# BradenDKelly/MetropolisMonteCarlo

Hardware: AMD Instinct MI355X
Metric: MC trial moves/sec (whole node), SPC/E NVT full Ewald fp64 (higher is better)
Workload: dtype f64

## Files before the change

### metropolismontecarlo_amd/csrc/mmc_batch.inc

```

#include <atomic>
#include <chrono>
#include <cmath>
#include <thread>

#define MMC_MAX_GROUPS 64
#define MMC_SERVER_AUTO_MAX 256
#define MMC_GEN_MAX 16
#define MMC_GEN_RING (MMC_GEN_MAX + 2)

struct mmc_batch {
    DeviceSystem sys;
    double lj_rcut = 0, qq_rcut = 0;
    int n_parts = 1;
    int kernel = 3;
    int server_wgs = -1;
    int wave_wgs = 0;
    int n_cus = 256;
    bool fast_ok = false;
    bool rigid_only = true;
    int image_by_molecule = -1;
    int zero_copy_moves = 0;
    MoveRec *h_moves[2] = { nullptr, nullptr };
    MoveRec *hd_moves[2] = { nullptr, nullptr };
    MoveRec *d_moves[2] = { nullptr, nullptr };
    PartOut *h_parts = nullptr, *d_parts = nullptr;
    int32_t *h_accept = nullptr, *d_accept = nullptr;
    int32_t *dev_accept = nullptr;
    int buf = 0;
    bool has_prev = false;
    std::vector<uint8_t> s_cur;
    std::vector<double> h_com, h_at;
    bool mirror_valid = false;
    int device_moves = 0;
    MoveRec *d_ring = nullptr;
    double *d_quat = nullptr;
    unsigned stamp = 0;
    int64_t steps_done = 0;
    int eval_parts = 0;
    int quat_mode = 0;
    double db[9] = { 0 };
    int persistent = -1;
    unsigned long long *h_ctrl = nullptr, *hd_ctrl = nullptr;
    unsigned long long *bar_ctrl = nullptr;
    int32_t *h_timeout = nullptr, *hd_timeout = nullptr;
    hipStream_t run_streams[MMC_MAX_GROUPS] = {};
    hipEvent_t run_events[MMC_MAX_GROUPS][4] = {};
    void *pool = nullptr;
    void (*pool_destroy)(void *) = nullptr;
    int steps_per_launch = 0;
    int accept_on_device = -1;
    DecideConsts *d_decide = nullptr;
    DecideConsts decide_host{};
    int server_stall_ms = 0;
    int64_t server_seq_offset = 0;
    bool needs_reload = false;
    std::vector<uint8_t> reloaded;
    int inject_torn = 0;
    bool vol_outstanding = false;
    bool vol_saved_fast_ok = false;
    int vol_saved_kernel = 0;
    std::vector<int32_t> pb_moved;
    int64_t trace_steps = 0;
    std::vector<double> trace_delta;
    std::vector<uint8_t> trace_flags;
    uint8_t *h_flags = nullptr, *hd_flags = nullptr, *d_flags = nullptr;
    uint8_t *bar_flags = nullptr;
    double2 *h_steps = nullptr, *hd_steps = nullptr, *d_steps = nullptr;
    void *widom_buf = nullptr;
    size_t widom_bytes = 0;
    void *widom_host = nullptr;
    size_t widom_host_bytes = 0;

    const MoveRec *dev_moves(int which) const
    {
        return zero_copy_moves ? hd_moves[which] : d_moves[which];
    }
};

static int32_t batch_pinned(void **h, void **d, size_t bytes)
{
    MMC_HIP(hipHostMalloc(h, bytes, hipHostMallocMapped | hipHostMallocCoherent));
    MMC_HIP(hipHostGetDevicePointer(d, *h, 0));
    memset(*h, 0, bytes);
    return MMC_OK;
}
// ... 167 lines not shown
        MMC_REQUIRE(value >= 0 && value <= (1 << 20), MMC_ERR_ARG, "wave_wgs outside 0..2^20");
        b->wave_wgs = (int)value;
    } else if (!strcmp(key, "server_wgs")) {
        MMC_REQUIRE(value >= -1 && value <= LAT_MAX_PARTS / LAT_WAVES && value != 1, MMC_ERR_ARG,
                    "server_wgs must be -1 (choose), 0 (one workgroup per replica) or 2..%d",
                    LAT_MAX_PARTS / LAT_WAVES);
        b->server_wgs = (int)value;
    } else if (!strcmp(key, "persistent")) {
        MMC_REQUIRE(value >= -1 && value <= 1, MMC_ERR_ARG, "persistent must be -1, 0 or 1");
        MMC_REQUIRE(!b->sys.pb.on || value != 1, MMC_ERR_UNSUPPORTED,
                    "per-replica boxes: the move server has one box");
        b->persistent = (int)value;
    } else if (!strcmp(key, "server_seq_offset")) {
        MMC_REQUIRE(value >= 0, MMC_ERR_ARG, "server_seq_offset must be >= 0");
        b->server_seq_offset = value;
    } else if (!strcmp(key, "server_stall_ms")) {
        MMC_REQUIRE(value >= 0 && value <= 10000, MMC_ERR_ARG, "server_stall_ms outside 0..10000");
        b->server_stall_ms = (int)value;
    } else if (!strcmp(key, "inject_torn")) {
        b->inject_torn = (int)value;
    } else if (!strcmp(key, "trace_steps")) {
        MMC_REQUIRE(value >= 0 && value * b->sys.R <= (1LL << 26), MMC_ERR_ARG, "trace_steps out of range");
        b->trace_steps = value;
    } else if (!strcmp(key, "zero_copy_moves")) {
        b->zero_copy_moves = value ? 1 : 0;
    } else if (!strcmp(key, "device_moves")) {
        MMC_REQUIRE(!b->sys.pb.on || value, MMC_ERR_UNSUPPORTED,
                    "per-replica boxes: the trial moves are drawn on the device");
        b->device_moves = value ? 1 : 0;
    } else if (!strcmp(key, "steps_per_launch")) {
        MMC_REQUIRE(value == 0 || value == 1 || value == 2 || value == 4 || value == 8 || value == 16, MMC_ERR_ARG,
                    "steps_per_launch must be 0 (by size), 1, 2, 4, 8 or 16");
        b->steps_per_launch = (int)value;
    } else if (!strcmp(key, "accept_on_device")) {
        MMC_REQUIRE(value >= -1 && value <= 1, MMC_ERR_ARG, "accept_on_device must be -1 (by size), 0 (host) or 1 (kernel)");
        b->accept_on_device = (int)value;
    } else if (!strcmp(key, "image_by_molecule")) {
        MMC_REQUIRE(value == -1 || value == 0, MMC_ERR_ARG, "image_by_molecule must be -1 (where valid) or 0 (never)");
        b->image_by_molecule = (int)value;
    } else {
        mmc_set_error("unknown option '%s'", key);
        return MMC_ERR_ARG;
    }
    return MMC_OK;
}

extern "C" int32_t mmc_batch_set_parts(mmc_batch *b, int32_t n_parts)
{
    return mmc_batch_set_option(b, "parts", n_parts);
}

extern "C" int32_t mmc_batch_set_replica(mmc_batch *b, int64_t r, const double *com,
                                         const double *coords)
{
    BATCH_CHECK(b);
    MMC_REQUIRE(!b->has_prev, MMC_ERR_STATE, "proposals outstanding: call mmc_batch_settle first");
    BATCH_NO_VOLUME_TRIAL(b);
    MMC_REQUIRE(com && coords, MMC_ERR_ARG, "NULL array argument");
    MMC_TRY(b->sys.set_replica(r, com, coords));
    if (b->needs_reload) {
        b->reloaded[r] = 1;
        bool all = true;
        for (uint8_t v : b->reloaded) all = all && v;
        if (all) {
            b->needs_reload = false;
            b->s_cur.assign(b->sys.R, 0);
// ... 46 lines not shown
    const int64_t n_mol = b->sys.n_mol;
    b->h_com.resize((size_t)b->sys.R * n_mol * 3);
    b->h_at.resize((size_t)b->sys.R * n_mol * 9);
    for (int64_t r = 0; r < b->sys.R; r++)
        MMC_TRY(b->sys.get_replica(r, &b->h_com[(size_t)r * n_mol * 3],
                                   &b->h_at[(size_t)r * n_mol * 9]));
    b->mirror_valid = true;
    return MMC_OK;
}

static inline void batch_mirror_commit(mmc_batch *b, int64_t r, const MoveRec &m)
{
    const int64_t n_mol = b->sys.n_mol;
    memcpy(&b->h_com[((size_t)r * n_mol + (m.mol - 1)) * 3], m.com_new, sizeof(double) * 3);
    memcpy(&b->h_at[((size_t)r * n_mol + (m.mol - 1)) * 9], m.atoms_new, sizeof(double) * 9);
}

static inline void batch_fill_old(mmc_batch *b, int64_t r, MoveRec &m)
{
    const int64_t n_mol = b->sys.n_mol;
    memcpy(m.com_old, &b->h_com[((size_t)r * n_mol + (m.mol - 1)) * 3], sizeof(double) * 3);
    memcpy(m.atoms_old, &b->h_at[((size_t)r * n_mol + (m.mol - 1)) * 9], sizeof(double) * 9);
}

struct DevGen {
    uint64_t seed;
    uint64_t replica0;
    int64_t rng_off;
    int64_t step;
    int n_gen;
    bool upload_steps;
};

static int32_t batch_ensure_ring(mmc_batch *b)
{
    if (!b->d_ring)
        MMC_TRY(b->sys.dmalloc((void **)&b->d_ring, sizeof(MoveRec) * MMC_GEN_RING * b->sys.R));
    return MMC_OK;
}

static inline const MoveRec *batch_ring_slot(const mmc_batch *b, int64_t step)
{
    return b->d_ring + (step % MMC_GEN_RING) * b->sys.R;
}

static int batch_kernel_for(const mmc_batch *b, int64_t nr, int P)
{
    if (b->sys.pb.on)
        return 1;
    return b->kernel != 3 ? b->kernel : (nr * P >= (int64_t)16 * b->n_cus ? 2 : 1);
}

struct DevDecide {
    const DecideConsts *dc;
    int64_t step;
    PartOut *parts;
    bool fetch_flags;
    int n_sub;
};

static int32_t batch_launch(mmc_batch *b, hipStream_t stream, int64_t r0, int64_t nr, int P,
                            int buf, bool has_prev, const PairParams &pp,
                            hipEvent_t before_kernel = nullptr, const DevGen *dg = nullptr,
                            unsigned stamp = 0, const DevDecide *dd = nullptr)
{
    DeviceSystem &s = b->sys;
    const MoveRec *cur, *prev;
    const uint8_t *flagv = nullptr;
    if (dg) {
        flagv = b->hd_flags;
        const double2 *stp = b->hd_steps;
        if (!b->zero_copy_moves) {
            if (dd ? dd->fetch_flags : !b->bar_flags)
                k_fetch_bytes<<<(unsigned)((nr + 1023) / 1024), 256, 0, stream>>>(
                    b->d_flags + r0, b->hd_flags + r0, (int)nr);
            if (dg->upload_steps)
                MMC_HIP(hipMemcpyAsync(b->d_steps + r0, b->h_steps + r0, sizeof(double2) * nr,
                                       hipMemcpyHostToDevice, stream));
            flagv = b->bar_flags && !dd ? b->bar_flags : b->d_flags;
            stp = b->d_steps;
        }
        if (dg->n_gen > 0) {
            GenArgs ga;
            ga.steps = stp; ga.seed = dg->seed; ga.replica0 = dg->replica0;
            ga.rng_off = dg->rng_off; ga.step0 = dg->step; ga.n_gen = dg->n_gen;
            ga.ring = MMC_GEN_RING; ga.ring_stride = s.R; ga.flag0 = flagv;
            ga.quat_mode = b->quat_mode;
            memcpy(ga.db, b->db, sizeof(ga.db));
            const int64_t n = nr * dg->n_gen;
            if (s.pb.on)
                k_propose<<<(unsigned)((n + 63) / 64), 64, 0, stream>>>(s.bv, s.rec, b->d_ring, ga, (int)r0,
                                                                        (int)nr, has_prev ? 1 : 0, s.pb_view());
            else
                k_propose<<<(unsigned)((n + 63) / 64), 64, 0, stream>>>(s.bv, s.rec, b->d_ring, ga,
                                                                        (int)r0, (int)nr, has_prev ? 1 : 0);
        }
        cur = batch_ring_slot(b, dg->step);
        prev = has_prev ? batch_ring_slot(b, dg->step + MMC_GEN_RING - 1) : nullptr;
    } else {
        b->rigid_only = false;
        s.r_mol_max = INFINITY;
        if (!b->zero_copy_moves)
            MMC_HIP(hipMemcpyAsync(b->d_moves[buf] + r0, b->h_moves[buf] + r0,
                                   sizeof(MoveRec) * nr, hipMemcpyHostToDevice, stream));
        cur = b->dev_moves(buf);
        prev = has_prev ? b->dev_moves(buf ^ 1) : nullptr;
    }
    if (before_kernel)
        MMC_HIP(hipEventRecord(before_kernel, stream));
    dim3 grid((unsigned)P, (unsigned)nr);
    MMC_REQUIRE(!dd || (dg && P == 1 && !b->zero_copy_moves && batch_kernel_for(b, nr, P) == 2), MMC_ERR_ASSERT,
                "the kernel's own accept decision needs device-side proposals, one part per move and the wave kernel");
    const int kernel = batch_kernel_for(b, nr, P);
    if (kernel == 4) {
        MMC_REQUIRE(lat_applies(4 * P, (int)s.n_mol, (int)s.nkvecs), MMC_ERR_UNSUPPORTED,
                    "kernel 4 needs 4..%d parts (a multiple of 4) with at most %d molecules per pair "
                    "part", LAT_MAX_PARTS, LAT_MAXMOL);
        k_move_eval_lat<<<grid, LAT_WAVES * 64, 0, stream>>>(s.bv, s.rec, s.qq_tab, s.kpack, s.fc,
                                                             cur, prev, b->d_parts, 4 * P, pp, (int)r0,
                                                             flagv, stamp);
    } else if (kernel == 2) {
        const int64_t n_units = nr * P;
        int64_t wgs = (n_units + WV_MWAVES - 1) / WV_MWAVES;
        const int64_t cap = b->wave_wgs > 0 ? b->wave_wgs : (int64_t)(4 * WV_OCC / WV_MWAVES) * b->n_cus;
        if (wgs > cap) wgs = cap;
        const bool img = dg && b->rigid_only && b->image_by_molecule != 0 &&
                         s.image_by_molecule(std::max(pp.lj_gate_sq, pp.qq_gate_sq)) &&
                         s.pairs_inside_slack(pp.qq_gate_sq, pp.qq_slack_sq) &&
                         s.pairs_inside_slack(pp.lj_gate_sq, pp.lj_slack_sq);
#define MMC_WAVE_LAUNCH(SUBST, IMG) MMC_WAVE_LAUNCH3(SUBST, IMG, false)
#define MMC_WAVE_LAUNCH3(SUBST, IMG, MULTI)                                                      \
    k_move_eval_wave<SUBST, IMG, MULTI><<<(unsigned)wgs, WV_MWAVES * 64, 0, stream>>>(            \
        s.bv, s.rec, s.qq_tab, s.kpack, s.fc, cur, prev, dd ? dd->parts : b->d_parts, P, pp,     \
        (int)r0, (int)n_units, flagv, stamp, dd ? dd->dc : nullptr, dd ? (long long)dd->step : 0LL,      \
        dd ? dd->n_sub : 1, (int)(dg ? dg->step % MMC_GEN_RING : 0))
        if (P == 1 && dd && dd->n_sub > 1) {
            if (img) MMC_WAVE_LAUNCH3(false, true, true); else MMC_WAVE_LAUNCH3(false, false, true);
        } else if (P == 1) {
            if (img) MMC_WAVE_LAUNCH(false, true); else MMC_WAVE_LAUNCH(false, false);
        } else {
            if (img) MMC_WAVE_LAUNCH(true, true); else MMC_WAVE_LAUNCH(true, false);
        }
#undef MMC_WAVE_LAUNCH
#undef MMC_WAVE_LAUNCH3
    } else if (kernel == 1 && s.pb.on)
        k_move_eval_fast<<<grid, MMC_BLOCK, 0, stream>>>(s.bv, s.rec, nullptr, s.kpack, s.fc, cur, prev,
                                                         b->d_parts, P, pp, (int)r0, flagv, stamp,
                                                         s.pb_view());
    else if (kernel == 1)
        k_move_eval_fast<<<grid, MMC_BLOCK, 0, stream>>>(s.bv, s.rec, s.qq_tab, s.kpack, s.fc, cur,
                                                         prev, b->d_parts, P, pp, (int)r0, flagv,
                                                         stamp);
    else
        k_move_eval<<<grid, MMC_BLOCK, 0, stream>>>(s.bv, cur, prev, b->d_parts, P, pp, (int)r0,
                                                    s.rec, flagv, stamp);
    MMC_HIP(hipGetLastError());
    return MMC_OK;
}

static int batch_server_parts(int64_t n_mol, int64_t R)
{
    int64_t pairs = (n_mol + 63) / 64;
    const int64_t cap = R == 1 ? 4 : SRV_WAVES - 1;
    if (pairs > cap) pairs = cap;
    if (pairs < 1) pairs = 1;
    return (int)pairs + 1;
}

// ... 421 lines not shown
```

### metropolismontecarlo_amd/csrc/mmc_engine.inc

```
#include <atomic>
#include <chrono>
#include <cmath>
#include <condition_variable>
#include <mutex>
#include <thread>

#ifndef MMC_HOST_CHUNK
#define MMC_HOST_CHUNK 128
#endif

namespace {

struct Rng {
    uint64_t s[4];
    static uint64_t splitmix(uint64_t &x)
    {
        uint64_t z = (x += 0x9e3779b97f4a7c15ULL);
        z = (z ^ (z >> 30)) * 0xbf58476d1ce4e5b9ULL;
        z = (z ^ (z >> 27)) * 0x94d049bb133111ebULL;
        return z ^ (z >> 31);
    }
    void seed(uint64_t v)
    {
        for (int k = 0; k < 4; k++)
// ... 96 lines not shown
    std::chrono::steady_clock::time_point t_post;
};

inline void adjust_step(int64_t &naccepp, int64_t &attempp, int64_t naccept, int64_t attempt,
                        double set_value, double L, double &d_max)
{
    if (attempp == 0) {
        naccepp = naccept;
        attempp = attempt;
        return;
    }
    if (attempt == attempp)
        return;
    const double ratio = (double)(naccept - naccepp) / (double)(attempt - attempp);
    const double dr_old = d_max;
    d_max = d_max * ratio / set_value;
    const double dr_ratio = d_max / dr_old;
    if (dr_ratio > 1.5) d_max = dr_old * 1.5;
    if (dr_ratio < 0.5) d_max = dr_old * 0.5;
    if (d_max > L / 2) d_max = L / 2;
    naccepp = naccept;
    attempp = attempt;
}

struct Driver {
    mmc_batch *b;
    const mmc_run_params *p;
    double *energies;
    mmc_chain *chains = nullptr;
    int adjust = 0;
    bool devgen = false;
    bool devacc = false;
    int K = 1;
    bool server = false;
    int server_waves = 0;
    int server_lat_wgs = 0;
    std::vector<Group> groups;
    std::vector<Rng> rng;
    std::vector<uint8_t> acc_prev, kind;
    PairParams pp;
    int P = 1, T = 1;
    SpinBarrier bar;
    std::atomic<int32_t> status{ MMC_OK };
    std::atomic<int> drained_polls{ 0 };
    char err[256] = "";
    std::vector<mmc_run_stats> tstats;
    std::vector<double> trace_t;
    std::chrono::steady_clock::time_point trace_t0;
    std::vector<double> entry_t;
    std::vector<double> mark_t;
    double now_us() const { return std::chrono::duration<double, std::micro>(std::chrono::steady_clock::now() - trace_t0).count(); }
    int64_t rng_off = 0;
    std::atomic<int> inject_left{ 0 };

    ChainKey chain_key(int64_t r) const
    {
        return ChainKey{ p->seed, (uint32_t)(p->replica0 + (uint64_t)r) };
    }

    int collect(int64_t r, unsigned want, PartOut *parts, int &q_done, mmc_run_stats &st, int slot = 0)
    {
        for (; q_done < P; q_done++) {
            const PartOut *src = &b->h_parts[(size_t)slot * b->sys.R + r * P + q_done];
            if (part_stamp_of(*(const volatile int32_t *)&src->ovl[1]) != want)
                return 0;
            std::atomic_thread_fence(std::memory_order_acquire);
// ... 84 lines not shown
                        c.rot_set_value, b->sys.box, c.dphi_max);
            if (devgen)
                b->h_steps[r] = make_double2(c.dr_max, c.dphi_max);
        }
    }

    void metropolis(const Group &g, int64_t lo, int64_t hi, int64_t step_done, mmc_run_stats &st,
                    bool gated = false, int slot = -1)
    {
        const unsigned want = (slot >= 0 ? g.stamp_of[slot] : g.stamp) & MMC_STAMP_MASK;
        const int sl = slot >= 0 ? slot : 0;
        if (gated && hi > lo) {
            const PartOut *gate = &b->h_parts[(size_t)sl * b->sys.R + (hi - 1) * P + (P - 1)];
            for (unsigned spins = 1; part_stamp_of(*(const volatile int32_t *)&gate->ovl[1]) != want; spins++) {
                if (((spins & 0xffff) == 0 && !still_running(g)) || status.load(std::memory_order_relaxed) != MMC_OK)
                    return;
                for (int k = 0; k < 16; k++)
                    mmc_cpu_relax();
            }
        }
        for (int64_t r = lo; r < hi; r++) {
            PartOut parts[MMC_MAX_PARTS];
            int q_done = 0;
            for (unsigned spins = 1;; spins++) {
                const int c = collect(r, want, parts, q_done, st, sl);
                if (c > 0)
                    break;
                if (c < 0 || ((spins & 0xfffff) == 0 && !still_running(g)))
                    return;
                mmc_cpu_relax();
            }
            const int64_t n_sub = slot >= 0 ? std::min<int64_t>(K, p->n_steps - step_done) : 1;
            if (n_sub > 1) {
                unsigned long long bits;
                memcpy(&bits, &parts[0].lj_pot[1], 8);
                const unsigned acc_mask = (unsigned)bits & 0xffffu, ovl_mask = (unsigned)(bits >> 16) & 0xffffu,
                               kind_mask = (unsigned)(bits >> 32) & 0xffffu;
                energies[r] += parts[0].lj_pot[0];
                for (int64_t k = 0; k < n_sub; k++) {
                    const int kd = (kind_mask >> k) & 1;
                    const bool acc = (acc_mask >> k) & 1;
                    if (kd == 0) { st.trans_attempt++; st.trans_accept += acc; }
                    else { st.rot_attempt++; st.rot_accept += acc; }
                    st.overlaps += (ovl_mask >> k) & 1;
                    if (acc && step_done + k + 1 < p->n_steps)
                        b->s_cur[r] ^= 1;
                    if (k + 1 == n_sub) {
                        acc_prev[r] = acc ? 1 : 0;
                        kind[r] = (uint8_t)kd;
                    }
                }
                st.moves += n_sub;
            } else if (slot >= 0) {
                kind[r] = (uint8_t)mmc_move_kind(chain_key(r), (uint64_t)(rng_off + step_done));
                decide(r, parts, step_done, st, part_accept_of(parts[0].ovl[1]));
                if (acc_prev[r] && step_done + 1 < p->n_steps)
                    b->s_cur[r] ^= 1;
            } else
                decide(r, parts, step_done, st);
        }
    }

    template <class F> void share(const Group &g, int t, F &&fn) const
    {
        const int64_t tail = g.nr >= 16 * (int64_t)MMC_HOST_CHUNK * T && !no_tail_share ? g.nr / tail_div : 0;
        const int64_t bulk = g.nr - tail;
        if (bulk * t / T < bulk * (t + 1) / T)
            fn(g.r0 + bulk * t / T, g.r0 + bulk * (t + 1) / T, false);
        const int64_t n_chunks = (tail + MMC_HOST_CHUNK - 1) / MMC_HOST_CHUNK;
        for (int64_t c = t; c < n_chunks; c += T) {
// ... 94 lines not shown
            timed = false;
        }
        return MMC_OK;
    }

    int32_t launch(Group &g, int64_t step, mmc_run_stats &st, hipStream_t on = nullptr)
    {
        g.launched_on = on ? on : g.stream;
        if (server) {
            const bool new_steps = step == 0 || (adjust && step % b->sys.n_mol == 0);
            g.n_launch++;
            g.timed = false;
            g.stamp = ++b->stamp;
            g.t_post = std::chrono::steady_clock::now();
            std::atomic_thread_fence(std::memory_order_release);
            if (b->server_stall_ms > 0 && step == 2)
                std::this_thread::sleep_for(std::chrono::milliseconds(b->server_stall_ms));
            for (int64_t r = g.r0; r < g.r0 + g.nr; r++)
                batch_server_post(b, r, step + 1, g.stamp,
                                  (unsigned)b->h_flags[r] | (new_steps ? SRV_STEPS : 0u));
            st.launches++;
            return MMC_OK;
        }
        DevGen dg{};
        if (devgen) {
            const int64_t n_mol = b->sys.n_mol, i0 = step % n_mol;
            dg.seed = p->seed;
            dg.replica0 = p->replica0;
            dg.rng_off = rng_off;
            dg.step = step;
            dg.upload_steps = step == 0 || (adjust && i0 == 0);
            if (step >= g.gen_end) {
                int64_t k = n_mol - 1 < 1 ? 1 : n_mol - 1;
                if (k > MMC_GEN_MAX) k = MMC_GEN_MAX;
                if (k > p->n_steps - step) k = p->n_steps - step;
                if (adjust && k > n_mol - i0) k = n_mol - i0;
                dg.n_gen = (int)k;
                g.gen_end = step + k;
            }
        }
        g.n_launch++;
        g.timed = p->time_kernels > 0
                  && (g.n_launch - 1) % (unsigned)p->time_kernels == (unsigned)p->time_kernels / 2;
        g.stamp = ++b->stamp;
        if (devacc) {
            const int64_t n_sub = std::min<int64_t>(K, p->n_steps - step);
            const int slot = (int)((step / K) & 1);
            g.stamp_of[slot] = g.stamp;
            g.timed_of[slot] = g.timed;
            DevDecide dd{ b->d_decide, rng_off + step, b->d_parts + (size_t)slot * b->sys.R, step == 0, (int)n_sub };
            MMC_TRY(batch_launch(b, g.launched_on, g.r0, g.nr, P, g.buf, step > 0, pp,
                                 g.timed ? g.evs[slot][0] : nullptr, &dg, g.stamp, &dd));
            if (g.timed)
                MMC_HIP(hipEventRecord(g.evs[slot][1], g.launched_on));
            g.timed = false;
            st.launches++;
            return MMC_OK;
        }
        MMC_TRY(batch_launch(b, g.launched_on, g.r0, g.nr, P, g.buf, g.has_prev, pp,
                             g.timed ? g.ev0 : nullptr, devgen ? &dg : nullptr, g.stamp));
        if (g.timed)
            MMC_HIP(hipEventRecord(g.ev1, g.launched_on));
        st.launches++;
        return MMC_OK;
    }

    void settle_slice(const Group &g, int64_t lo, int64_t hi)
    {
        const MoveRec *prev = b->h_moves[g.buf];
        for (int64_t r = lo; r < hi; r++) {
            b->h_accept[r] = acc_prev[r];
            if (acc_prev[r]) {
                b->s_cur[r] ^= 1;
                if (!devgen)
                    batch_mirror_commit(b, r, prev[r]);
            }
        }
    }
    int32_t settle_enqueue(Group &g)
    {
        return batch_settle_range(b, g.stream, g.r0, g.nr,
                                  devgen ? batch_ring_slot(b, p->n_steps - 1) : b->dev_moves(g.buf), false);
    }
// ... 454 lines not shown
        }
        if (p->time_kernels) {
            for (int k = 0; k < 4; k++)
                if (!b->run_events[g][k])
                    MMC_HIP(hipEventCreate(&b->run_events[g][k]));
            d.groups[g].ev0 = b->run_events[g][0];
            d.groups[g].ev1 = b->run_events[g][1];
            for (int k = 0; k < 4; k++)
                d.groups[g].evs[k / 2][k % 2] = b->run_events[g][k];
        }
    }
    d.devacc = d.devgen && !d.server && d.P == 1 && !b->zero_copy_moves && !(chains && adjust);
    int64_t nr_max = 0;
    for (const Group &g : d.groups) {
        d.devacc = d.devacc && batch_kernel_for(b, g.nr, d.P) == 2;
        nr_max = std::max(nr_max, g.nr);
    }
    {
        int want = b->accept_on_device;
        if (getenv("MMC_DEVICE_ACCEPT")) want = 1;
        if (getenv("MMC_HOST_ACCEPT")) want = 0;
        const bool multi_ok = !chains && b->trace_steps == 0 && s.n_mol > MMC_GEN_MAX && b->steps_per_launch != 1;
        if (want < 0)
            want = (multi_ok || nr_max > (int64_t)4096 * d.T) ? 1 : 0;
        d.devacc = d.devacc && want == 1;
    }
    d.K = 1;
    if (d.devacc && !chains && b->trace_steps == 0 && s.n_mol > MMC_GEN_MAX) {
        d.K = b->steps_per_launch > 0 ? b->steps_per_launch : 8;
        if (const char *e = getenv("MMC_STEPS_PER_LAUNCH"))
            d.K = atoi(e);
        if (d.K != 1 && d.K != 2 && d.K != 4 && d.K != 8 && d.K != 16)
            d.K = 1;
    }
    if (d.devacc) {
        MMC_TRY(batch_ensure_ring(b));
        DecideConsts dc{};
        dc.temperature = p->temperature; dc.factor = s.bv.factor;
        dc.seed = p->seed; dc.replica0 = (uint32_t)p->replica0;
        dc.flags = b->d_flags;
        dc.ring = b->d_ring; dc.ring_slots = MMC_GEN_RING; dc.ring_stride = s.R;
        if (!b->d_decide)
            MMC_TRY(s.dmalloc((void **)&b->d_decide, sizeof(DecideConsts)));
        if (memcmp(&dc, &b->decide_host, sizeof(dc)) != 0) {
            MMC_HIP(hipMemcpy(b->d_decide, &dc, sizeof(dc), hipMemcpyHostToDevice));
            b->decide_host = dc;
        }
        if (const char *e = getenv("MMC_RUN_AHEAD"))
            d.run_ahead = atoi(e) ? 1 : 0;
        if (const char *e = getenv("MMC_LAUNCH_AT"))
            d.launch_at = std::min(1.0, std::max(0.0, atof(e) / 100.0));
    }
    if (d.server)
        for (Group &g : d.groups)
            g.stream = d.groups[0].stream;
    if (d.server)
        MMC_TRY(batch_server_start(b, d.groups[0].stream, d.server_waves, d.pp, p->seed, p->replica0,
                                   b->steps_done, d.server_lat_wgs));
    d.rng.resize(d.devgen ? 0 : R);
    for (int64_t r = 0; r < (d.devgen ? 0 : R); r++) {
        uint64_t h = p->seed;
        h = Rng::splitmix(h) ^ (p->replica0 + (uint64_t)r);
        h = Rng::splitmix(h) ^ (uint64_t)b->steps_done;
        d.rng[r].seed(h);
    }
    d.acc_prev.assign(R, 0);
    d.kind.assign(R, 0);
    b->trace_delta.assign((size_t)(b->trace_steps * R), 0.0);
    b->trace_flags.assign((size_t)(b->trace_steps * R), 0);
    d.tstats.assign(d.T, mmc_run_stats{});
    if (d.server) {
        d.server_stamp0 = b->stamp;
        b->stamp += (unsigned)p->n_steps;
    }

    const auto t0 = std::chrono::steady_clock::now();
// ... 74 lines not shown
    }
    stats->server_steps = d.server ? p->n_steps : 0;
    stats->device_decisions = d.devacc ? stats->moves : 0;
    if (d.server)
        stats->launches = p->n_steps * (int64_t)d.groups.size();
    stats->wall_ms = std::chrono::duration<double, std::milli>(t1 - t0).count();
    for (int64_t r = 0; r < R; r++)
        stats->energy_sum += chains ? chains[r].energy : energies[r];
    for (size_t g = 0; g < d.groups.size(); g++)
        if (d.groups[g].stream)
            (void)hipStreamSynchronize(d.groups[g].stream);
    if (run_trace) {
        const auto t2 = std::chrono::steady_clock::now();
        auto us = [](std::chrono::steady_clock::duration x) { return std::chrono::duration<double, std::micro>(x).count(); };
        fprintf(stderr, "run trace: threads %.0f us, final settle %.0f us (enqueued after %.0f), last sync %.0f us; launches at",
                us(t_join - t_enter), us(t1 - t_join), us(t_enq - t_join), us(t2 - t1));
        for (double x : d.trace_t)
            fprintf(stderr, " %.0f", x);
        fprintf(stderr, "\nrun trace: threads entered at");
        for (double x : d.entry_t)
            fprintf(stderr, " %.0f", x);
        fprintf(stderr, "\nrun trace: thread 0 per (step, group) [after barrier, after its share, (same), after barrier]:");
        for (size_t k = 0; k < d.mark_t.size(); k++)
            fprintf(stderr, "%s%.0f", k % 4 == 0 ? " | " : " ", d.mark_t[k]);
        fprintf(stderr, "\n");
    }
    b->buf = 0;
    b->has_prev = false;
    b->inject_torn = 0;
    if (status == MMC_OK)
        b->steps_done += p->n_steps;
    else {
        b->needs_reload = true;
        b->reloaded.assign(R, 0);
    }
    return status;
}

extern "C" int32_t mmc_batch_run(mmc_batch *b, const mmc_run_params *p, double *energies,
                                 mmc_run_stats *stats)
{
    MMC_REQUIRE(energies, MMC_ERR_ARG, "NULL argument");
    return run_impl(b, p, energies, nullptr, 0, stats);
}

extern "C" int32_t mmc_batch_run_chains(mmc_batch *b, const mmc_run_params *p, mmc_chain *chains,
                                        int32_t adjust, mmc_run_stats *stats)
{
    MMC_REQUIRE(chains, MMC_ERR_ARG, "NULL argument");
    if (b)
        BATCH_ONE_BOX(b, "mmc_batch_run_chains");
    if (b)
        for (int64_t r = 0; r < b->sys.R; r++)
            MMC_REQUIRE(chains[r].dr_max >= 0 && chains[r].dphi_max >= 0
                            && (!adjust || (chains[r].trans_set_value > 0 && chains[r].rot_set_value > 0)),
                        MMC_ERR_ARG, "chain %lld: bad step sizes / set values", (long long)r);
    return run_impl(b, p, nullptr, chains, adjust, stats);
}

extern "C" int32_t mmc_batch_run_npt(mmc_batch *b, const mmc_run_params *p, const mmc_npt_params *q,
                                     double *energy, mmc_run_stats *stats, mmc_npt_stats *ns)
{
    BATCH_CHECK(b);
    BATCH_ONE_BOX(b, "mmc_batch_run_npt (per-replica boxes: mmc_batch_run_npt_replicas)");
    MMC_REQUIRE(p && q && energy && stats && ns, MMC_ERR_ARG, "NULL argument");
    MMC_REQUIRE(b->sys.R == 1, MMC_ERR_UNSUPPORTED,
// ... 89 lines not shown
```

### metropolismontecarlo_amd/csrc/mmc_kernels.hpp

```cpp
#pragma once
#include "mmc_device.hpp"

struct BatchView {
    double *comx, *comy, *comz;
    double *ax, *ay, *az;
    int64_t mol_stride, atom_stride;
    const int32_t *first0, *cnt, *atype;
    const double *charge, *eps, *sig;
    int32_t n_mol, n_atoms, n_types;
    double box;
    double *S;
    int64_t nk_stride;
    const int32_t *kxyz;
    const double *cfac;
    const int16_t *kmap;
    int32_t nkvecs, nk;
    double kappa, factor;
    uint16_t *comq;
    int64_t cq_stride;
    double *quat;
};

__host__ __device__ inline uint16_t com_quant(double x, double inv_box)
{
// ... 360 lines not shown
    h += dpp_row_shr<2>(h);
    h += dpp_row_shr<4>(h);
    return part_checksum_fold((uint32_t)__builtin_amdgcn_readlane(h, 7));
}

__device__ inline double pack_ovl(int o0, int o1, unsigned stamp, uint32_t csum, int accept = 0)
{
    const unsigned lo = (csum << 1) | (unsigned)(o0 & 1),
                   hi = ((unsigned)(accept & 1) << 31) | ((stamp & MMC_STAMP_MASK) << 1) | (unsigned)(o1 & 1);
    return __longlong_as_double((long long)(((unsigned long long)hi << 32) | lo));
}
__host__ __device__ inline uint32_t part_stamp_of(int32_t ovl1) { return ((uint32_t)ovl1 >> 1) & MMC_STAMP_MASK; }
__host__ __device__ inline int part_accept_of(int32_t ovl1) { return (int)((uint32_t)ovl1 >> 31); }

__host__ __device__ inline double mmc_move_delta(const double *w7, bool ov_old, bool ov_new, double factor)
{
    const double e0 = (0.0 + w7[0]) * 4, e1 = (0.0 + w7[1]) * 4;
    double q0 = ov_old ? 0.0 : 0.0 + w7[4], q1 = ov_new ? 0.0 : 0.0 + w7[5];
    q0 *= factor; q1 *= factor;
    const double d_recip = (ov_old || ov_new) ? 0.0 : (0.0 + w7[6]) * factor;
    return ((e1 - e0) + (q1 - q0)) + d_recip;
}

struct MoveRec;
struct DecideConsts {
    double temperature, factor;
    uint64_t seed;
    uint32_t replica0;
    int32_t ring_slots;
    const MoveRec *ring;
    int64_t ring_stride;
    uint8_t *flags;
};
#define MMC_STEPS_PER_LAUNCH_MAX 16

__global__ __launch_bounds__(MMC_BLOCK) void k_move_eval(BatchView bv, const MoveRec *cur,
                                                         const MoveRec *prev, PartOut *out,
                                                         int n_parts, PairParams pp, int r_base,
                                                         double *rec, const uint8_t *flagv,
                                                         unsigned stamp)
{
    __shared__ __align__(16) double pobuf[8];
    __shared__ Chosen ch;
    __shared__ Pending pd;
    __shared__ int32_t list[MMC_LIST_CAP];
    __shared__ int32_t wcnt[MMC_WAVES];
    __shared__ double red[6 * MMC_WAVES];
    __shared__ cplx tab[2][3][3][MMC_NKTAB];

    const int r = r_base + blockIdx.y, part = blockIdx.x, tid = threadIdx.x;
    const SysView s = sys_view(bv, r);
    const MoveRec *mv = cur + r;
    const int flags = flagv ? (int)flagv[r] : mv->flags;
    const bool commit = prev && (flags & 1);
    const int scur = (flags >> 1) & 1;
    const int i0 = mv->mol - 1;
    const int pend = commit ? prev[r].mol - 1 : -1;

    if (tid == 0) {
        pd.mol = pend;
        ch.i0 = i0; ch.na = 3;
    }
    if (commit && tid < 12) {
        if (tid < 3) pd.com[tid] = prev[r].com_new[tid];
        else pd.at[(tid - 3) / 3][(tid - 3) % 3] = prev[r].atoms_new[tid - 3];
    }
    __syncthreads();
// ... 261 lines not shown
```

### metropolismontecarlo_amd/csrc/mmc_wave.hpp

```cpp
#pragma once
#include "mmc_fast.hpp"
#include "mmc_propose.hpp"

#ifndef WV_WAVES
#define WV_WAVES 4
#endif
#ifndef WV_OCC
#define WV_OCC 5
#endif
#ifndef WV_MWAVES
#define WV_MWAVES WV_WAVES
#endif
#ifndef WV_LIST
#define WV_LIST 640
#endif
#ifndef WV_PF
#define WV_PF 6
#endif
#define MMC_CQ_PAD (4 * 64 * (2 * WV_PF + 2))
#ifndef WV_TPF
#define WV_TPF 3
#endif

typedef uint16_t wv_list_t;
// ... 100 lines not shown
    const cplx e1 = { cs, sn }, one = { 1.0, 0.0 };
    row[5] = one;
    row[6] = e1;
    row[4] = c_conj(e1);
    cplx p = e1;
#pragma unroll
    for (int k = 2; k <= 5; k++) {
        p = c_mul(p, e1);
        row[5 + k] = p;
        row[5 - k] = c_conj(p);
    }
}

__device__ __forceinline__ int wave_decide(const double *outw, bool ov_old, bool ov_new,
                                           const DecideConsts *__restrict__ dc, long long step, int r,
                                           int scur, int lane, double *delta_out = nullptr, bool store_flags = true)
{
    const double delta = mmc_move_delta(outw, ov_old, ov_new, dc->factor);
    if (delta_out)
        *delta_out = delta;
    const double x = delta / dc->temperature;
    const double u = mmc_metropolis_uniform(ChainKey{ dc->seed, dc->replica0 + (uint32_t)r }, (uint64_t)step);
    bool met;
    if (x < 0.0) met = true;
    else if (1.0 - x > u + 1e-9) met = true;
    else if ((1.0 + x) * u > 1.0 + 1e-9) met = false;
    else met = exp(-x) > u;
    const int acc = (met && !(ov_old || ov_new)) ? 1 : 0;
    if (store_flags && lane == 0)
        dc->flags[r] = (uint8_t)(acc | ((scur ^ acc) << 1));
    return acc;
}

template <bool SUBST, bool IMG, bool MULTI = false>
__global__ __launch_bounds__(WV_MWAVES * 64) __attribute__((amdgpu_waves_per_eu(WV_OCC, WV_OCC))) void k_move_eval_wave(
    BatchView bv, double *rec, const double *__restrict__ qq_tab,
    const int32_t *__restrict__ kpack, FastConsts fc, const MoveRec *__restrict__ cur,
    const MoveRec *__restrict__ prev, PartOut *out, int n_parts, PairParams pp, int r_base,
    int n_units, const uint8_t *flagv, unsigned stamp, const DecideConsts *__restrict__ dc, long long dec_step,
    int n_sub_arg, int slot0)
{
    const int n_sub = MULTI ? n_sub_arg : 1;
    __shared__ __align__(16) WaveSharedT<WV_MWAVES> sm;
    const int tid = threadIdx.x, lane0 = tid & 63;
    const int wv = __builtin_amdgcn_readfirstlane(tid >> 6);

    for (int k = tid; k < MMC_QQ_TABLE_DOUBLES; k += WV_MWAVES * 64)
        sm.qtab[k] = qq_tab[k];
    __syncthreads();

    const int n_mol = bv.n_mol, nkv = bv.nkvecs;
    const double box = bv.box;
    const BoxConsts bc = box_consts(box);
    const int np = (n_parts == 1) ? 1 : n_parts - 1;
    const int plen = (n_mol + np - 1) / np;
    const bool same_gate = pp.lj_gate_sq == pp.qq_gate_sq;
    const double inv_box = uniform_f64(1.0 / box);
    uint32_t gate_q;
    asm volatile("v_readfirstlane_b32 %0, %1" : "=s"(gate_q) : "v"(com_quant_gate(fmax(pp.lj_gate_sq, pp.qq_gate_sq), box)));
    wv_list_t *const list = sm.list[wv];
    const double *const pvw = sm.pvw[wv];

    for (int unit = blockIdx.x * WV_MWAVES + wv; unit < n_units; unit += gridDim.x * WV_MWAVES) {
        int lane = lane0;
        if (!MULTI)
            asm volatile("" : "+v"(lane));
        int rl = unit, part = 0;
        if (n_parts != 1) {
            rl = unit / n_parts;
            part = unit - rl * n_parts;
        }
        const int r = r_base + rl;
        const bool do_pairs = (n_parts == 1) || (part < n_parts - 1);
        const bool do_recip = (n_parts == 1) || (part == n_parts - 1);
        const int j_begin = do_pairs ? min(part * plen, n_mol) : 0;
        const int j_end = do_pairs ? min(j_begin + plen, n_mol) : 0;
        double *const myrec = rec + (int64_t)r * n_mol * MMC_RSTRIDE;

        int flags_carry = -1;
        double e_sum = 0.0;
        unsigned acc_mask = 0, ovl_mask = 0, kind_mask = 0;
      for (int sub = 0; sub < n_sub; sub++) {
        if (MULTI) {
            lane = lane0;
            asm volatile("" : "+v"(lane));
        }
        const MoveRec *cur_s = cur, *prev_s = prev;
        if (n_sub > 1) {
            const int sl = (slot0 + sub) % dc->ring_slots, slp = (slot0 + sub + dc->ring_slots - 1) % dc->ring_slots;
            cur_s = dc->ring + (int64_t)sl * dc->ring_stride;
            if (sub > 0)
                prev_s = dc->ring + (int64_t)slp * dc->ring_stride;
        }
        WV_STAMP(0);
        const double *mvp = reinterpret_cast<const double *>(cur_s + r);
        double w = 0.0;
// ... 30 lines not shown
                }
            }
            if (bv.quat) {
                const double q0 = wave_pick(pw, 13), q1 = wave_pick(pw, 14),
                             q2 = wave_pick(pw, 15), q3 = wave_pick(pw, 16);
                if (part == 0 && lane >= 13 && lane < 17)
                    quat_commit(bv, r, pend, lane - 13, pw, q0 * q0 + q1 * q1 + q2 * q2 + q3 * q3 > 0.25);
            }
            wave_sync();
        }

#define WV_CQ_BASE (bv.comq + (int64_t)r * 3 * bv.cq_stride)
#define WV_PART_DST (out + (int64_t)r * n_parts + part)
        auto decide_here = [&](bool o0, bool o1) -> int {
            if (!dc)
                return 0;
            if (n_sub <= 1)
                return wave_decide(sm.outw[wv], o0, o1, dc, dec_step, r, scur, lane);
            double delta;
            const bool last = sub + 1 == n_sub;
            const int acc = wave_decide(sm.outw[wv], o0, o1, dc, dec_step + sub, r, scur, lane, &delta, last);
            if (acc) {
                e_sum += delta;
                acc_mask |= 1u << sub;
            }
            if (o0 || o1)
                ovl_mask |= 1u << sub;
            kind_mask |= (unsigned)((lane_i32((int)(hdr >> 32), 0) >> 8) & 1) << sub;
            flags_carry = acc | ((scur ^ acc) << 1);
            if (last) {
                wave_sync();
                if (lane < 7)
                    sm.outw[wv][lane] = lane == 0 ? e_sum
                                 : lane == 1 ? __longlong_as_double((long long)(acc_mask | (ovl_mask << 16)) | ((long long)kind_mask << 32)) : 0.0;
                wave_sync();
            }
            return acc;
        };
#define WV_DECIDE(o0, o1) decide_here(o0, o1)
#define WV_RECORD_OVL(o) (n_sub > 1 ? false : (o))
#define WV_STORE_IF (sub + 1 == n_sub)
#define WV_STORE_SYSTEM MULTI
#define WV_ZERO opaque_f64(0.0)
#define WV_SUBST SUBST
#define WV_IMG IMG
#ifndef WV_XY_MOVE
#define WV_XY_MOVE 1
#endif
#define WV_XY WV_XY_MOVE
#define WV_PASSES 2
#define WV_AFTER_PHASE_TABLES                                                                    \
    if (!SUBST && commit)                                                                        \
        asm volatile("s_waitcnt vmcnt(0)" ::: "memory");
#include "mmc_wave_unit.inc"
#undef WV_AFTER_PHASE_TABLES
#undef WV_IMG
#undef WV_PASSES
#undef WV_XY
#undef WV_SUBST
#undef WV_ZERO
#undef WV_CQ_BASE
#undef WV_PART_DST
#undef WV_DECIDE
#undef WV_RECORD_OVL
#undef WV_STORE_IF
#undef WV_STORE_SYSTEM
        if (n_sub > 1)
// ... 446 lines not shown
```

Baseline: 143.2 million.

## Add whole-call multi-step launches and atomic work queue for wave kernel

Adds a whole_call option that sets the per-launch step count to the whole call (up to 32 steps, capped by molecule count). It grows the proposal ring to match and widens the accept/overlap/kind bitmasks from 16 to 32 bits. It also adds an atomic ticket queue so waves in the multi-step kernel pull units dynamically instead of using a fixed grid stride, which balances uneven per-replica work. The intent is fewer launches and less tail imbalance. The cost is a global atomic per unit, plus ring reallocation and queue resets that need device syncs.

```diff
diff --git a/metropolismontecarlo_amd/csrc/mmc_batch.inc b/metropolismontecarlo_amd/csrc/mmc_batch.inc
--- a/metropolismontecarlo_amd/csrc/mmc_batch.inc
+++ b/metropolismontecarlo_amd/csrc/mmc_batch.inc
@@ -8,6 +8,7 @@
 #define MMC_SERVER_AUTO_MAX 256
 #define MMC_GEN_MAX 16
 #define MMC_GEN_RING (MMC_GEN_MAX + 2)
+#define MMC_QUEUE_STRIDE 32
 
 struct mmc_batch {
     DeviceSystem sys;
@@ -34,6 +35,7 @@
     bool mirror_valid = false;
     int device_moves = 0;
     MoveRec *d_ring = nullptr;
+    int ring_slots = MMC_GEN_RING;
     double *d_quat = nullptr;
     unsigned stamp = 0;
     int64_t steps_done = 0;
@@ -49,9 +51,13 @@
     void *pool = nullptr;
     void (*pool_destroy)(void *) = nullptr;
     int steps_per_launch = 0;
+    int whole_call = 0;
     int accept_on_device = -1;
     DecideConsts *d_decide = nullptr;
     DecideConsts decide_host{};
+    unsigned *d_queue = nullptr;
+    unsigned queue_base[MMC_MAX_GROUPS] = {};
+    bool queue_reset = false;
     int server_stall_ms = 0;
     int64_t server_seq_offset = 0;
     bool needs_reload = false;
@@ -285,6 +291,9 @@
         MMC_REQUIRE(value == 0 || value == 1 || value == 2 || value == 4 || value == 8 || value == 16, MMC_ERR_ARG,
                     "steps_per_launch must be 0 (by size), 1, 2, 4, 8 or 16");
         b->steps_per_launch = (int)value;
+    } else if (!strcmp(key, "whole_call")) {
+        MMC_REQUIRE(value == 0 || value == 1, MMC_ERR_ARG, "whole_call must be 0 (launches of steps_per_launch) or 1 (one per call)");
+        b->whole_call = (int)value;
     } else if (!strcmp(key, "accept_on_device")) {
         MMC_REQUIRE(value >= -1 && value <= 1, MMC_ERR_ARG, "accept_on_device must be -1 (by size), 0 (host) or 1 (kernel)");
         b->accept_on_device = (int)value;
@@ -397,16 +406,26 @@
     bool upload_steps;
 };
 
-static int32_t batch_ensure_ring(mmc_batch *b)
-{
-    if (!b->d_ring)
-        MMC_TRY(b->sys.dmalloc((void **)&b->d_ring, sizeof(MoveRec) * MMC_GEN_RING * b->sys.R));
+static int32_t batch_ensure_ring(mmc_batch *b, int slots = MMC_GEN_RING)
+{
+    if (b->d_ring && b->ring_slots >= slots)
+        return MMC_OK;
+    if (b->d_ring) {
+        MMC_HIP(hipDeviceSynchronize());
+        std::vector<void *> &a = b->sys.allocs;
+        a.erase(std::remove(a.begin(), a.end(), (void *)b->d_ring), a.end());
+        MMC_HIP(hipFree(b->d_ring));
+        b->d_ring = nullptr;
+    }
+    slots = std::max(slots, (int)MMC_GEN_RING);
+    MMC_TRY(b->sys.dmalloc((void **)&b->d_ring, sizeof(MoveRec) * (size_t)slots * b->sys.R));
+    b->ring_slots = slots;
     return MMC_OK;
 }
 
 static inline const MoveRec *batch_ring_slot(const mmc_batch *b, int64_t step)
 {
-    return b->d_ring + (step % MMC_GEN_RING) * b->sys.R;
+    return b->d_ring + (step % b->ring_slots) * b->sys.R;
 }
 
 static int batch_kernel_for(const mmc_batch *b, int64_t nr, int P)
@@ -422,6 +441,8 @@
     PartOut *parts;
     bool fetch_flags;
     int n_sub;
+    unsigned *queue;
+    unsigned queue_base;
 };
 
 static int32_t batch_launch(mmc_batch *b, hipStream_t stream, int64_t r0, int64_t nr, int P,
@@ -449,7 +470,7 @@
             GenArgs ga;
             ga.steps = stp; ga.seed = dg->seed; ga.replica0 = dg->replica0;
             ga.rng_off = dg->rng_off; ga.step0 = dg->step; ga.n_gen = dg->n_gen;
-            ga.ring = MMC_GEN_RING; ga.ring_stride = s.R; ga.flag0 = flagv;
+            ga.ring = b->ring_slots; ga.ring_stride = s.R; ga.flag0 = flagv;
             ga.quat_mode = b->quat_mode;
             memcpy(ga.db, b->db, sizeof(ga.db));
             const int64_t n = nr * dg->n_gen;
@@ -461,7 +482,7 @@
                                                                         (int)r0, (int)nr, has_prev ? 1 : 0);
         }
         cur = batch_ring_slot(b, dg->step);
-        prev = has_prev ? batch_ring_slot(b, dg->step + MMC_GEN_RING - 1) : nullptr;
+        prev = has_prev ? batch_ring_slot(b, dg->step + b->ring_slots - 1) : nullptr;
     } else {
         b->rigid_only = false;
         s.r_mol_max = INFINITY;
@@ -498,7 +519,8 @@
     k_move_eval_wave<SUBST, IMG, MULTI><<<(unsigned)wgs, WV_MWAVES * 64, 0, stream>>>(            \
         s.bv, s.rec, s.qq_tab, s.kpack, s.fc, cur, prev, dd ? dd->parts : b->d_parts, P, pp,     \
         (int)r0, (int)n_units, flagv, stamp, dd ? dd->dc : nullptr, dd ? (long long)dd->step : 0LL,      \
-        dd ? dd->n_sub : 1, (int)(dg ? dg->step % MMC_GEN_RING : 0))
+        dd ? dd->n_sub : 1, (int)(dg ? dg->step % b->ring_slots : 0), dd ? dd->queue : nullptr,      \
+        dd ? dd->queue_base : 0u)
         if (P == 1 && dd && dd->n_sub > 1) {
             if (img) MMC_WAVE_LAUNCH3(false, true, true); else MMC_WAVE_LAUNCH3(false, false, true);
         } else if (P == 1) {
diff --git a/metropolismontecarlo_amd/csrc/mmc_engine.inc b/metropolismontecarlo_amd/csrc/mmc_engine.inc
--- a/metropolismontecarlo_amd/csrc/mmc_engine.inc
+++ b/metropolismontecarlo_amd/csrc/mmc_engine.inc
@@ -152,6 +152,7 @@
     bool devgen = false;
     bool devacc = false;
     int K = 1;
+    int gen_max = MMC_GEN_MAX;
     bool server = false;
     int server_waves = 0;
     int server_lat_wgs = 0;
@@ -302,10 +303,11 @@
             }
             const int64_t n_sub = slot >= 0 ? std::min<int64_t>(K, p->n_steps - step_done) : 1;
             if (n_sub > 1) {
-                unsigned long long bits;
+                unsigned long long bits, kbits;
                 memcpy(&bits, &parts[0].lj_pot[1], 8);
-                const unsigned acc_mask = (unsigned)bits & 0xffffu, ovl_mask = (unsigned)(bits >> 16) & 0xffffu,
-                               kind_mask = (unsigned)(bits >> 32) & 0xffffu;
+                memcpy(&kbits, &parts[0].lj_vir[0], 8);
+                const unsigned acc_mask = (unsigned)bits, ovl_mask = (unsigned)(bits >> 32),
+                               kind_mask = (unsigned)kbits;
                 energies[r] += parts[0].lj_pot[0];
                 for (int64_t k = 0; k < n_sub; k++) {
                     const int kd = (kind_mask >> k) & 1;
@@ -466,7 +468,7 @@
             dg.upload_steps = step == 0 || (adjust && i0 == 0);
             if (step >= g.gen_end) {
                 int64_t k = n_mol - 1 < 1 ? 1 : n_mol - 1;
-                if (k > MMC_GEN_MAX) k = MMC_GEN_MAX;
+                if (k > gen_max) k = gen_max;
                 if (k > p->n_steps - step) k = p->n_steps - step;
                 if (adjust && k > n_mol - i0) k = n_mol - i0;
                 dg.n_gen = (int)k;
@@ -482,7 +484,11 @@
             const int slot = (int)((step / K) & 1);
             g.stamp_of[slot] = g.stamp;
             g.timed_of[slot] = g.timed;
-            DevDecide dd{ b->d_decide, rng_off + step, b->d_parts + (size_t)slot * b->sys.R, step == 0, (int)n_sub };
+            const size_t gi = (size_t)(&g - groups.data());
+            DevDecide dd{ b->d_decide, rng_off + step, b->d_parts + (size_t)slot * b->sys.R, step == 0, (int)n_sub,
+                          n_sub > 1 ? b->d_queue + MMC_QUEUE_STRIDE * gi : nullptr, b->queue_base[gi] };
+            if (n_sub > 1)
+                b->queue_base[gi] += (unsigned)(g.nr * P);
             MMC_TRY(batch_launch(b, g.launched_on, g.r0, g.nr, P, g.buf, step > 0, pp,
                                  g.timed ? g.evs[slot][0] : nullptr, &dg, g.stamp, &dd));
             if (g.timed)
@@ -1003,16 +1009,28 @@
             d.K = atoi(e);
         if (d.K != 1 && d.K != 2 && d.K != 4 && d.K != 8 && d.K != 16)
             d.K = 1;
+        if (b->whole_call == 1) {
+            d.K = (int)std::min<int64_t>(std::min<int64_t>(p->n_steps, MMC_STEPS_PER_LAUNCH_MAX), s.n_mol - 1);
+            d.gen_max = std::max(d.K, (int)MMC_GEN_MAX);
+        }
     }
     if (d.devacc) {
-        MMC_TRY(batch_ensure_ring(b));
+        MMC_TRY(batch_ensure_ring(b, d.gen_max + 2));
         DecideConsts dc{};
         dc.temperature = p->temperature; dc.factor = s.bv.factor;
         dc.seed = p->seed; dc.replica0 = (uint32_t)p->replica0;
         dc.flags = b->d_flags;
-        dc.ring = b->d_ring; dc.ring_slots = MMC_GEN_RING; dc.ring_stride = s.R;
+        dc.ring = b->d_ring; dc.ring_slots = b->ring_slots; dc.ring_stride = s.R;
         if (!b->d_decide)
             MMC_TRY(s.dmalloc((void **)&b->d_decide, sizeof(DecideConsts)));
+        if (!b->d_queue || b->queue_reset) {
+            if (!b->d_queue)
+                MMC_TRY(s.dmalloc((void **)&b->d_queue, sizeof(unsigned) * MMC_QUEUE_STRIDE * MMC_MAX_GROUPS));
+            MMC_HIP(hipMemset(b->d_queue, 0, sizeof(unsigned) * MMC_QUEUE_STRIDE * MMC_MAX_GROUPS));
+            MMC_HIP(hipDeviceSynchronize());
+            memset(b->queue_base, 0, sizeof(b->queue_base));
+            b->queue_reset = false;
+        }
         if (memcmp(&dc, &b->decide_host, sizeof(dc)) != 0) {
             MMC_HIP(hipMemcpy(b->d_decide, &dc, sizeof(dc), hipMemcpyHostToDevice));
             b->decide_host = dc;
@@ -1153,6 +1171,7 @@
         b->steps_done += p->n_steps;
     else {
         b->needs_reload = true;
+        b->queue_reset = true;
         b->reloaded.assign(R, 0);
     }
     return status;
diff --git a/metropolismontecarlo_amd/csrc/mmc_kernels.hpp b/metropolismontecarlo_amd/csrc/mmc_kernels.hpp
--- a/metropolismontecarlo_amd/csrc/mmc_kernels.hpp
+++ b/metropolismontecarlo_amd/csrc/mmc_kernels.hpp
@@ -416,7 +416,7 @@
     int64_t ring_stride;
     uint8_t *flags;
 };
-#define MMC_STEPS_PER_LAUNCH_MAX 16
+#define MMC_STEPS_PER_LAUNCH_MAX 32
 
 __global__ __launch_bounds__(MMC_BLOCK) void k_move_eval(BatchView bv, const MoveRec *cur,
                                                          const MoveRec *prev, PartOut *out,
diff --git a/metropolismontecarlo_amd/csrc/mmc_wave.hpp b/metropolismontecarlo_amd/csrc/mmc_wave.hpp
--- a/metropolismontecarlo_amd/csrc/mmc_wave.hpp
+++ b/metropolismontecarlo_amd/csrc/mmc_wave.hpp
@@ -156,13 +156,21 @@
     return acc;
 }
 
+__device__ __forceinline__ int wave_ticket(unsigned *queue, unsigned base, int n_waves, int lane)
+{
+    unsigned t = 0;
+    if (lane == 0)
+        t = atomicAdd(queue, 1u);
+    return n_waves + (int)(__builtin_amdgcn_readfirstlane(t) - base);
+}
+
 template <bool SUBST, bool IMG, bool MULTI = false>
 __global__ __launch_bounds__(WV_MWAVES * 64) __attribute__((amdgpu_waves_per_eu(WV_OCC, WV_OCC))) void k_move_eval_wave(
     BatchView bv, double *rec, const double *__restrict__ qq_tab,
     const int32_t *__restrict__ kpack, FastConsts fc, const MoveRec *__restrict__ cur,
     const MoveRec *__restrict__ prev, PartOut *out, int n_parts, PairParams pp, int r_base,
     int n_units, const uint8_t *flagv, unsigned stamp, const DecideConsts *__restrict__ dc, long long dec_step,
-    int n_sub_arg, int slot0)
+    int n_sub_arg, int slot0, unsigned *queue, unsigned queue_base)
 {
     const int n_sub = MULTI ? n_sub_arg : 1;
     __shared__ __align__(16) WaveSharedT<WV_MWAVES> sm;
@@ -185,7 +193,9 @@
     wv_list_t *const list = sm.list[wv];
     const double *const pvw = sm.pvw[wv];
 
-    for (int unit = blockIdx.x * WV_MWAVES + wv; unit < n_units; unit += gridDim.x * WV_MWAVES) {
+    for (int unit = blockIdx.x * WV_MWAVES + wv; unit < n_units;
+         unit = MULTI && queue ? wave_ticket(queue, queue_base, gridDim.x * WV_MWAVES, lane0)
+                               : unit + gridDim.x * WV_MWAVES) {
         int lane = lane0;
         if (!MULTI)
             asm volatile("" : "+v"(lane));
@@ -282,7 +292,8 @@
                 wave_sync();
                 if (lane < 7)
                     sm.outw[wv][lane] = lane == 0 ? e_sum
-                                 : lane == 1 ? __longlong_as_double((long long)(acc_mask | (ovl_mask << 16)) | ((long long)kind_mask << 32)) : 0.0;
+                                 : lane == 1 ? __longlong_as_double((long long)acc_mask | ((long long)ovl_mask << 32))
+                                 : lane == 2 ? __longlong_as_double((long long)kind_mask) : 0.0;
                 wave_sync();
             }
             return acc;
```

After: 146.8 million (median of 6 runs). 2.5% higher.
